# cvg/nicer-slam

Hardware: AMD Instinct MI355X
Metric: rays/sec (fwd+bwd), one tracking iteration (higher is better)
Workload: dtype f32; 1 GPU; Replica room0 tracking iteration, 1024 rays x 128 samples (+640 sampler evaluations/ray), single MI355X, fp32 [BASELINE configs[1]]; rays_per_gpu=1024, samples_per_ray=128, sampler_evals_per_ray=640, global_rays=1024, engine=fused, param_grads=False, hip_graph=True, driver=KernelTracker, python_gc=off inside the timed regions (as timeit), ray_chunks=1, cache_prewarm_steps=100, cache_prewarm_batches=disjoint from the warm-up and timed batches, parallelism=single, rccl_ranks=0, full=False

## Files before the change

### include/nicer_slam_amd.h

```cpp
#ifndef NICER_SLAM_AMD_H
#define NICER_SLAM_AMD_H

#include <stdint.h>

#ifdef __cplusplus
extern "C" {
#endif

#define NSA_OK 0
#define NSA_EUNSUPPORTED_C 1
#define NSA_ETOO_MANY_LEVELS 2
#define NSA_ELAUNCH 3
#define NSA_EBADARG 4
#define NSA_EUNSUPPORTED_NET 5
#define NSA_EMESH_TOO_LARGE 6

#define NSA_MAX_LEVELS 32

typedef void *nsa_stream_t;

const char *nsa_strerror(int code);
int nsa_version(void);


// ... 140 lines not shown
                   float beta1, float beta2, float eps, uint32_t lr_step, float lr_gamma, const float *loss, float *best,
                   nsa_stream_t stream);
int nsa_track_begin(const float *uv_in, const float *gt_in, float *uv, float *gt, const float *K, const float *cam, uint32_t n,
                    float *pose, float *rays_o, float *rays_d, float *depth_scale, nsa_stream_t stream);
int nsa_track_begin_draw(const float *uv_in, const float *gt_in, float *uv, float *gt, const float *K, const float *cam, uint32_t n,
                         float *pose, float *rays_o, float *rays_d, float *depth_scale, uint64_t *state, uint64_t n_rand,
                         float *t_rand, uint32_t E, uint32_t n_extra, uint32_t S, int32_t *extra_idx, nsa_stream_t stream);
int nsa_composite_track(const float *rays_o, const float *rays_d, const float *z_vals, const float *sdf, const float *rgb,
                        const float *voxels, uint32_t voxel_res, uint32_t R, uint32_t S, const float *gt, uint32_t n_total,
                        float *rgb_values, float *ray_loss, float *g_sdf, float *g_rgb, float *g_grad, nsa_stream_t stream);
int nsa_track_finish(const float *uv, const float *K, float *cam, uint32_t n, uint32_t S, const float *z_vals, const float *g_x,
                     const float *g_dir, const float *ray_loss, float *g_cam, int do_adam, float reduce_weight, float *exp_avg,
                     float *exp_avg_sq, float *step, float lr, float beta1, float beta2, float eps, uint32_t lr_step,
                     float lr_gamma, float *best, float *workspace, nsa_stream_t stream);
uint64_t nsa_track_finish_workspace(uint32_t n);
int nsa_adam_step_scaled(float *param, const float *grad, const float *grad_div, float *exp_avg, float *exp_avg_sq,
                         float *step, uint32_t n, float lr, float beta1, float beta2, float eps, uint32_t lr_step,
                         float lr_gamma, const float *loss, float *best, nsa_stream_t stream);


int nsa_morton_keys(const nsa_points_t *pts, int32_t *keys, nsa_stream_t stream);

int nsa_morton_order(const nsa_points_t *pts, int32_t *order, uint32_t *workspace, uint32_t key_bits, nsa_stream_t stream);
uint64_t nsa_morton_order_workspace(uint32_t P);

int nsa_update_voxels(const nsa_points_t *pts, float *voxels, uint32_t res, nsa_stream_t stream);

int nsa_adam_table_step(float *param, const float *grad, float *exp_avg, float *exp_avg_sq, uint64_t n, uint32_t step,
                        float lr, float beta1, float beta2, float eps, nsa_stream_t stream);

// ... 139 lines not shown
```

### nicer_slam_amd/_native.py

```python
import ctypes
import os

import torch

_TAG = os.environ.get("NSA_LIB_TAG", "")
_LIB_PATH = os.path.join(os.path.dirname(os.path.abspath(__file__)), "lib",
                         "libnicer_slam_amd" + ("_" + _TAG if _TAG else "") + ".so")

if not os.path.exists(_LIB_PATH):
    raise ImportError(
        f"{_LIB_PATH} not found: the HIP extension has not been built.  Run "
        "`python -m nicer_slam_amd.build` (needs hipcc; cross-compiles gfx950 without a GPU).")

lib = ctypes.CDLL(_LIB_PATH)

_p, _u32, _f32, _i = ctypes.c_void_p, ctypes.c_uint32, ctypes.c_float, ctypes.c_int

lib.nsa_strerror.restype = ctypes.c_char_p
lib.nsa_strerror.argtypes = [_i]
lib.nsa_version.restype = _i
lib.nsa_hash_encode_forward.restype = _i
lib.nsa_hash_encode_forward.argtypes = [_p, _p, _p, _p, _u32, _u32, _u32, _u32, _f32, _u32, _i, _p, _p]
lib.nsa_hash_encode_backward.restype = _i
lib.nsa_hash_encode_backward.argtypes = [_p, _p, _p, _p, _p, _u32, _u32, _u32, _u32, _f32, _u32, _i, _p, _p, _p]
# ... 179 lines not shown
lib.nsa_track_tail.argtypes = [_p, _p, _p, _u32, _p, _p, _p, _i, _f32, _p, _p, _p, _f32, _f32, _f32, _f32, _u32, _f32, _p, _p,
                               _p]
EXPORTS += ["nsa_track_head", "nsa_track_tail"]
lib.nsa_track_begin.restype = _i
lib.nsa_track_begin.argtypes = [_p, _p, _p, _p, _p, _p, _u32, _p, _p, _p, _p, _p]
lib.nsa_composite_track.restype = _i
lib.nsa_composite_track.argtypes = [_p, _p, _p, _p, _p, _p, _u32, _u32, _u32, _p, _u32, _p, _p, _p, _p, _p, _p]
lib.nsa_track_finish.restype = _i
lib.nsa_track_finish.argtypes = [_p, _p, _p, _u32, _u32, _p, _p, _p, _p, _p, _i, _f32, _p, _p, _p, _f32, _f32, _f32, _f32, _u32,
                                 _f32, _p, _p, _p]
lib.nsa_track_finish_workspace.restype = ctypes.c_uint64
lib.nsa_track_finish_workspace.argtypes = [_u32]
lib.nsa_track_begin_draw.restype = _i
lib.nsa_track_begin_draw.argtypes = [_p, _p, _p, _p, _p, _p, _u32, _p, _p, _p, _p, _p, ctypes.c_uint64, _p, _u32, _u32, _u32, _p, _p]
EXPORTS += ["nsa_track_begin", "nsa_track_begin_draw", "nsa_composite_track", "nsa_track_finish", "nsa_track_finish_workspace"]

lib.nsa_morton_keys.restype = _i
lib.nsa_morton_keys.argtypes = [_pp, _p, _p]
lib.nsa_morton_order.restype = _i
lib.nsa_morton_order.argtypes = [_pp, _p, _p, _u32, _p]
lib.nsa_morton_order_workspace.restype = ctypes.c_uint64
lib.nsa_morton_order_workspace.argtypes = [_u32]
EXPORTS += ["nsa_morton_order", "nsa_morton_order_workspace"]
EXPORTS += ["nsa_morton_keys"]

lib.nsa_adam_step_scaled.restype = _i
lib.nsa_adam_step_scaled.argtypes = [_p, _p, _p, _p, _p, _p, _u32, _f32, _f32, _f32, _f32, _u32, _f32, _p, _p, _p]
EXPORTS += ["nsa_adam_step_scaled"]


# ... 46 lines not shown
```

### nicer_slam_amd/csrc/render_sdfnet4.hip

```cpp
#include <cstdlib>
#include "sdf_net4.hpp"

namespace nsa {

#ifndef NSA_NW4_FWD
#define NSA_NW4_FWD 4
#endif
#ifndef NSA_NW4_BWD
#define NSA_NW4_BWD 8
#endif
#ifndef NSA_NW4_PAIR
#define NSA_NW4_PAIR 8
#endif
constexpr int stage_floats4(int nw) { return nw >= 8 ? 9216 : 6144; }

struct SdfNet4Args {
    PointSrc src;
    const float* table;
    const float* wp;
    float divide_factor;
    int accumulate;
    float* sdf;
    float* grad;
    float* feat;
// ... 282 lines not shown
    __shared__ LevelGeom s_geom[16];
    stage16_begin<Seq, Seq::NW, Seq::BUF>(stage, a.wp);
    geom_to_lds(geom, s_geom);
    const int lane = threadIdx.x & 63;
    const int j = lane & 15, q = lane >> 4;
    uint32_t tile = blockIdx.x * Seq::NW + (threadIdx.x >> 6);
    const uint32_t n_tiles = (a.src.P + 15) / 16;
    const bool wave_live = tile < n_tiles;
    if (!wave_live) tile = n_tiles - 1;
#define NSA_BODY_SYNC __syncthreads();
#include "sdfnet4_bwd_body.inc"
#undef NSA_BODY_SYNC
    TS_MARK(10)
    TS_END
}

static_assert(NSA_NW4_BWD * 64 * (2 * 8 + 1) <= stage_floats4(NSA_NW4_BWD), "scatter scratch must fit the idle stage buffer");

#if NSA_PIECES == 1
template <int LC, int CC, int NHC, int LF, int CF, int NHF>
__global__ __launch_bounds__(64 * NSA_NW4_PAIR, NSA_OCC4_FWD) void k_sdfnet4_fwd_pair_res(SdfNet4PairArgs a, GridGeom16 gc, GridGeom16 gf) {
    using Seq = ResidentSeq<SdfOpsPair<NHC, NHF>>;
    __shared__ __attribute__((aligned(16))) float stage[res_off<Seq>(Seq::n)];
    __shared__ LevelGeom s_geom[32];
    resident_load<Seq, Seq::NW>(stage, a.wp_c, a.wp_f);
    if (threadIdx.x < 16) s_geom[threadIdx.x] = gc.lv[threadIdx.x];
    else if (threadIdx.x < 32) s_geom[threadIdx.x] = gf.lv[threadIdx.x - 16];
    stage_wait();
    const int lane = threadIdx.x & 63;
    const int j = lane & 15, q = lane >> 4;
// ... 127 lines not shown
                           (hipStream_t)stream, a, gc, gf);
        return launch_end();
    }
#endif
    hipLaunchKernelGGL((k_sdfnet4_fwd_pair<4, 8, 1, 8, 4, 3>), dim3((tiles + NSA_NW4_PAIR - 1) / NSA_NW4_PAIR), dim3(64 * NSA_NW4_PAIR), 0,
                       (hipStream_t)stream, a, gc, gf);
    return launch_end();
}

#ifdef NSA_X_TS
int NSA_ENTRY(nsa_debug_set_ts)(unsigned long long* p) {
    return hipMemcpyToSymbol(HIP_SYMBOL(nsa::g_ts4), &p, sizeof(p)) == hipSuccess ? 0 : 3;
}
#endif

int NSA_ENTRY(nsa_sdfnet4_emit_rows)(uint32_t n_hidden) {
    return n_hidden == 1 ? nsa::SE4<1>::ROWS : n_hidden == 3 ? nsa::SE4<3>::ROWS : -1;
}

}
```

### nicer_slam_amd/csrc/sdfnet4_bwd_body.inc

```
    uint32_t pid = tile * 16 + j;
    const bool live = wave_live && pid < a.src.P;
    if (pid >= a.src.P) pid = a.src.P - 1;
    const uint32_t pt = point_of(a.src, pid);
    float x[3], z;
    uint32_t ray;
    load_point(a.src, pt, x, ray, z);
    NSA_BODY_SYNC
    TS_MARK(4)
    constexpr int kJac = (8 / C) * 3 * C;
    __shared__ float jac_lds[Seq::NW * kJac * 64];
    float* jstore = jac_lds + (threadIdx.x >> 6) * (kJac * 64) + lane;
    float in[QIN];
    pe_slots4(x, q, in);
    grid_slots4<L, C>(x, a.divide_factor, a.table, s_geom, q, in, jstore);
    const bool emit = MAP && a.emit != nullptr && wave_live;
    const Emitter4 em{emit ? a.emit + (size_t)tile * 16 + j : nullptr, a.emit_ld, live};
    float sg[NH][QHS], hl[QHS];
    TS_MARK(5)
    hidden_forward4<NH, Seq>(stage, 0, a.wp, lane, q, in, sg, hl, emit ? &em : nullptr);
    TS_MARK(6)
    float dh[NH > 1 ? NH - 1 : 1][QHS], dl[QIN];
    reverse_pass4<NH, Seq>(stage, NH, a.wp, lane, q, sg, dh, dl, emit ? &em : nullptr);
    TS_MARK(7)
    if (emit) {
// ... 89 lines not shown
    float hb0[QIN];
    {
        f32x4v a6[6];
#pragma unroll
        for (int t = 0; t < 6; ++t) a6[t] = f32x4v{0.0f, 0.0f, 0.0f, 0.0f};
        gemm16_staged<Seq, Seq::NW, Seq::BUF, 2, 6>(stage, a.wp, 4 * NH, lane, ab, a6, nullptr, &ab_bound);
#pragma unroll
        for (int s = 0; s < QIN; ++s) hb0[s] = a6[s >> 2][s & 3];
    }
    float gx[3];
    slots_to_x_jac4<L, C>(a.divide_factor, jstore, q, in, hb0, gx);
    constexpr int kIdle = (Seq::n_parts() - 1) & 1 ? 0 : 1;
    if (MAP && a.g_table)
        table_grad_scatter4<L, C>(x, a.divide_factor, s_geom, q, lane, live, hb0, dl, nbar, a.g_table,
                                  stage + kIdle * Seq::BUF + (threadIdx.x >> 6) * 64 * (2 * C + 1));
#pragma unroll
    for (int d = 0; d < 3; ++d) gx[d] = quad_sum(gx[d] + xb2[d]);
    if (live && q == 0) {
#pragma unroll
        for (int d = 0; d < 3; ++d) {
            float v = gx[d];
            if (a.accumulate) v += a.g_x[(size_t)pt * 3 + d];
            a.g_x[(size_t)pt * 3 + d] = v;
        }
    }
```

### nicer_slam_amd/csrc/track_tail.hip

```cpp
#include "grid_common.hpp"
#include "draw_common.hpp"

namespace nsa {

__device__ __forceinline__ void cam_to_pose(const float* __restrict__ q, float* __restrict__ P) {
    const float r = q[0], i = q[1], j = q[2], k = q[3];
    const float s = 2.0f / (r * r + i * i + j * j + k * k);
    P[0] = -s * (j * j + k * k) + 1.0f;  P[1] = s * (i * j - k * r);          P[2] = s * (i * k + j * r);           P[3] = q[4];
    P[4] = s * (i * j + k * r);          P[5] = -s * (i * i + k * k) + 1.0f;  P[6] = s * (j * k - i * r);           P[7] = q[5];
    P[8] = s * (i * k - j * r);          P[9] = s * (j * k + i * r);          P[10] = -s * (i * i + j * j) + 1.0f;  P[11] = q[6];
    P[12] = 0.0f; P[13] = 0.0f; P[14] = 0.0f; P[15] = 1.0f;
}

__global__ void k_cam_to_pose(const float* __restrict__ cam, float* __restrict__ pose, uint32_t b) {
    const uint32_t n = blockIdx.x * blockDim.x + threadIdx.x;
    if (n >= b) return;
    cam_to_pose(cam + 7 * n, pose + 16 * n);
}

__device__ __forceinline__ void pose_grad_to_cam(const float* __restrict__ q, const float* __restrict__ G, float* __restrict__ o) {
    const float r = q[0], i = q[1], j = q[2], k = q[3];
    const float nn = r * r + i * i + j * j + k * k;
    const float s = 2.0f / nn;
    const float N[9] = {-(j * j + k * k), i * j - k * r, i * k + j * r, i * j + k * r, -(i * i + k * k), j * k - i * r,
                        i * k - j * r, j * k + i * r, -(i * i + j * j)};
    float A = 0.0f;
#pragma unroll
// ... 99 lines not shown
}

struct TrackArgs {
    const float* uv;
    const float* K;
    float* cam;
    float* pose;
    uint32_t n;
    float* rays_o; float* rays_d; float* depth_scale;
    const float* g_o; const float* g_d;
    float* g_cam;
    float reduce_weight;
    AdamArgs adam;
};

__device__ __forceinline__ void lift_pixel_k(const float* __restrict__ K, float u, float v, float (&c)[3]) {
    const float fx = K[0], sk = K[1], cx = K[2], fy = K[5], cy = K[6];
    c[0] = (u - cx + cy * sk / fy - sk * v / fy) / fx;
    c[1] = (v - cy) / fy;
    c[2] = 1.0f;
}

__global__ __launch_bounds__(256) void k_track_head(TrackArgs a) {
    const uint32_t r = blockIdx.x * 256 + threadIdx.x;
    float P[16];
    cam_to_pose(a.cam, P);
    if (r == 0) {
#pragma unroll
        for (int i = 0; i < 16; ++i) a.pose[i] = P[i];
    }
    if (r >= a.n) return;
    float c[3];
    lift_pixel_k(a.K, a.uv[2 * r], a.uv[2 * r + 1], c);
    float v[3];
#pragma unroll
    for (int k = 0; k < 3; ++k) {
        const float w = P[4 * k] * c[0] + P[4 * k + 1] * c[1] + P[4 * k + 2] * c[2] + P[4 * k + 3];
// ... 73 lines not shown
    }
}

struct FinishArgs {
    TrackArgs t;
    const float* z_vals;
    const float* g_x;
    const float* g_dir;
    const float* ray_loss;
    uint32_t S;
    float inv_n;
    float* part;
    unsigned* ticket;
};

constexpr int FIN_Q = 13;

__device__ __forceinline__ void track_begin_block(const TrackArgs& a, const float* uv_in, const float* gt_in, float* uv, float* gt,
                                                  const uint32_t bid) {
    const uint32_t r = bid * 256 + threadIdx.x;
    float P[16];
    cam_to_pose(a.cam, P);
    if (r == 0) {
#pragma unroll
        for (int i = 0; i < 16; ++i) a.pose[i] = P[i];
    }
    if (r >= a.n) return;
    const float pu = uv_in[2 * r], pv = uv_in[2 * r + 1];
    uv[2 * r] = pu;
    uv[2 * r + 1] = pv;
#pragma unroll
    for (int k = 0; k < 3; ++k) gt[3 * r + k] = gt_in[3 * r + k];
// ... 8 lines not shown
    }
    const float s = v[0] * v[0] + v[1] * v[1] + v[2] * v[2];
#pragma unroll
    for (int k = 0; k < 3; ++k) a.rays_d[3 * r + k] = v[k] / s;
    a.depth_scale[r] = c[2] / (c[0] * c[0] + c[1] * c[1] + c[2] * c[2]);
}

__global__ __launch_bounds__(256) void k_track_begin(TrackArgs a, const float* uv_in, const float* gt_in, float* uv, float* gt) {
    track_begin_block(a, uv_in, gt_in, uv, gt, blockIdx.x);
}

__global__ __launch_bounds__(256) void k_track_begin_draw(TrackArgs a, const float* uv_in, const float* gt_in, float* uv, float* gt,
                                                          DrawArgs d, uint32_t begin_blocks) {
    if (blockIdx.x < begin_blocks) track_begin_block(a, uv_in, gt_in, uv, gt, blockIdx.x);
    else draw_block(d, blockIdx.x - begin_blocks, gridDim.x - begin_blocks);
}

constexpr int FIN_W = 16;

__global__ __launch_bounds__(64 * FIN_W) void k_track_finish(FinishArgs f) {
    __shared__ float rp[FIN_W][FIN_Q];
    __shared__ float G[16];
    __shared__ unsigned last;
    const TrackArgs& a = f.t;
    const int lane = threadIdx.x & 63, wv = threadIdx.x >> 6;
    const uint32_t ray = blockIdx.x * FIN_W + wv;
    float P[16];
    cam_to_pose(a.cam, P);
    float t0 = 0.0f, m0 = 0.0f, v0 = 0.0f, p0 = 0.0f;
    if (a.adam.p && threadIdx.x < 7) {
        t0 = a.adam.step[0];
        m0 = a.adam.m[threadIdx.x];
        v0 = a.adam.v[threadIdx.x];
        p0 = a.adam.p[threadIdx.x];
    }
    const float best0 = (a.adam.p && a.adam.best && threadIdx.x == 0) ? a.adam.best[0] : 0.0f;
    float vals[FIN_Q];
#pragma unroll
    for (int q = 0; q < FIN_Q; ++q) vals[q] = 0.0f;
    if (ray < a.n) {
        float acc[6] = {0, 0, 0, 0, 0, 0};
        for (uint32_t i = lane; i < f.S; i += 64) {
            const size_t p = (size_t)ray * f.S + i;
            const float z = f.z_vals[p];
#pragma unroll
            for (int c = 0; c < 3; ++c) {
                const float gx = f.g_x[p * 3 + c];
                acc[c] += gx;
                acc[3 + c] += z * gx + f.g_dir[p * 3 + c];
            }
        }
#pragma unroll
        for (int q = 0; q < 6; ++q) {
#pragma unroll
            for (int off = 32; off > 0; off >>= 1) acc[q] += __shfl_xor(acc[q], off);
        }
        float c[3], v[3];
        lift_pixel_k(a.K, a.uv[2 * ray], a.uv[2 * ray + 1], c);
#pragma unroll
        for (int k = 0; k < 3; ++k) {
            const float w = P[4 * k] * c[0] + P[4 * k + 1] * c[1] + P[4 * k + 2] * c[2] + P[4 * k + 3];
            v[k] = w - P[4 * k + 3];
        }
        const float s = v[0] * v[0] + v[1] * v[1] + v[2] * v[2];
        const float vg = v[0] * acc[3] + v[1] * acc[4] + v[2] * acc[5];
#pragma unroll
        for (int k = 0; k < 3; ++k) {
            const float vb = acc[3 + k] / s - 2.0f * v[k] * vg / (s * s);
#pragma unroll
            for (int j = 0; j < 3; ++j) vals[4 * k + j] = vb * c[j];
            vals[4 * k + 3] = acc[k];
        }
        vals[12] = f.ray_loss[ray];
    }
    if (lane == 0) {
#pragma unroll
        for (int q = 0; q < FIN_Q; ++q) rp[wv][q] = vals[q];
    }
    __syncthreads();
    if (wv == 0) {
        if (lane < FIN_Q) {
            float x = 0.0f;
#pragma unroll
            for (int w = 0; w < FIN_W; ++w) x += rp[w][lane];
            __hip_atomic_store(f.part + (size_t)blockIdx.x * 16 + lane, x, __ATOMIC_RELAXED, __HIP_MEMORY_SCOPE_AGENT);
        }
        __threadfence();
// ... 21 lines not shown
        }
        __syncthreads();
        if (lane == 0) {
#pragma unroll
            for (int q = 0; q < FIN_Q; ++q) rp[wv][q] = x[q];
        }
        __syncthreads();
        if (threadIdx.x < FIN_Q) {
            float g = 0.0f;
#pragma unroll
            for (int w = 0; w < FIN_W; ++w) g += rp[w][threadIdx.x];
            G[threadIdx.x] = g;
        }
    }
    __syncthreads();
    __shared__ float msg[9], stepped[8];
    if (threadIdx.x == 0) {
        f.ticket[0] = 0u;
        float o[8];
        pose_grad_to_cam(a.cam, G, o);
        o[7] = G[12] * f.inv_n;
        const float w = a.reduce_weight > 0.0f ? a.reduce_weight : 1.0f;
#pragma unroll
        for (int i = 0; i < 8; ++i) { msg[i] = o[i] * w; a.g_cam[i] = msg[i]; }
        if (a.reduce_weight > 0.0f) a.g_cam[8] = a.reduce_weight;
    }
    __syncthreads();
    if (a.adam.p) {
        const float t = t0 + 1.0f;
        if (threadIdx.x < 7) stepped[threadIdx.x] = adam_one(a.adam, threadIdx.x, t, m0, v0, p0, msg[threadIdx.x]);
        __syncthreads();
        if (threadIdx.x == 0) {
            a.adam.step[0] = t;
            if (a.adam.best && msg[7] < best0) {
                a.adam.best[0] = msg[7];
                for (int i = 0; i < 7; ++i) a.adam.best[1 + i] = stepped[i];
            }
        }
    }
}

}

extern "C" {

int nsa_cam_to_pose(const float* cam, uint32_t b, float* pose, nsa_stream_t stream) {
    using namespace nsa;
    if (b == 0) return NSA_OK;
    if (!cam || !pose) return NSA_EBADARG;
    launch_begin();
    hipLaunchKernelGGL(k_cam_to_pose, dim3((b + 63) / 64), dim3(64), 0, (hipStream_t)stream, cam, pose, b);
    return launch_end();
}

// ... 110 lines not shown
    FinishArgs f{};
    f.t.uv = uv; f.t.K = K; f.t.cam = cam; f.t.n = n; f.t.g_cam = g_cam; f.t.reduce_weight = reduce_weight;
    if (do_adam) f.t.adam = AdamArgs{cam, g_cam, exp_avg, exp_avg_sq, step, nullptr, 7, lr, beta1, beta2, eps, lr_gamma, lr_step,
                                      best, g_cam + 7, nullptr};
    f.z_vals = z_vals; f.g_x = g_x; f.g_dir = g_dir; f.ray_loss = ray_loss; f.S = S;
    f.inv_n = 1.0f / (float)(3 * (uint64_t)n);
    const uint32_t blocks = (n + FIN_W - 1) / FIN_W;
    f.ticket = reinterpret_cast<unsigned*>(workspace);
    f.part = workspace + 4;
    launch_begin();
    hipLaunchKernelGGL(k_track_finish, dim3(blocks), dim3(64 * FIN_W), 0, (hipStream_t)stream, f);
    return launch_end();
}

}
```

### nicer_slam_amd/fused/render.py

```python
import ctypes
import os

import torch

from .._native import lib, check, PointsDesc
from ..hashencoder.backend import _timed
from . import pack
from .sampler import COLOUR_COARSE_BWD, COLOUR_FWD_TRACK, forward_pair_ok, grid_desc, packed_sdf, precision_of, sdf_grid_desc, tile_of


def hl_size(P):
    return ((P + 31) // 32) * 2048


def save_size(P):
    return ((P + 31) // 32) * (4096 + 256)


def hl_index(P, device):
    pid = torch.arange(P, device=device).unsqueeze(1)
    f = torch.arange(64, device=device).unsqueeze(0)
    tile, p = pid // 32, pid % 32
    t, rho = f // 32, f % 32
    h = (rho >> 2) & 1
# ... 106 lines not shown
        return b
    with _timed("k_colour_fwd", P * 16 * 8 * 2 * 4):
        check(lib.nsa_colour_forward(ctypes.byref(pts), ctypes.byref(gr), pr.data_ptr(), b["grad"].data_ptr(),
                                     b["feat"].data_ptr(), b["rgb"].data_ptr(),
                                     b["save"].data_ptr() if need_bwd else None, st))
    if not composite:
        return b
    with _timed("k_composite_fwd", P * 32):
        check(lib.nsa_composite_forward(rays_o.data_ptr(), rays_d.data_ptr(), z_vals.data_ptr(), b["sdf"].data_ptr(),
                                        b["rgb"].data_ptr(), b["grad"].data_ptr(), b["vox"].data_ptr(), model.voxel_res,
                                        R, S, b["weights"].data_ptr(), b["rgb_values"].data_ptr(), b["depth"].data_ptr(),
                                        b["nmap"].data_ptr(), b["entropy"].data_ptr(), st))
    return b


def composite_backward_raw(model, rays_o, rays_d, z_vals, b, stage, color_stage, g_rgbv=None, g_depth=None, g_nmap=None,
                           g_ent=None, g_w=None, params=None, track=None, reduce_rays=True):
    R, S = z_vals.shape
    P = R * S
    dev = z_vals.device
    imp = model.implicit_network
    gc, keep_c = sdf_grid_desc(model, "coarse")
    gf, keep_f = sdf_grid_desc(model, "fine")
    gr, keep_r = grid_desc(model.rendering_network.encoding, model.rendering_network.divide_factor, 2, precision_of(model, "colour"))
    pc, pf, pr = b["packs"]
    order = b.get("order")
    pts = _pts(rays_o, rays_d, z_vals, order)
    st = _stream()
    ptr = lambda t: None if t is None else t.data_ptr()
    gs = [None if g is None else g.contiguous() for g in (g_rgbv, g_depth, g_nmap, g_ent, g_w)]
    done = b.get("track_out") if track is not None else None
    g_sdf = done["g_sdf"] if done else torch.empty(P, device=dev)
    g_rgb = done["g_rgb"] if done else torch.empty(P, 3, device=dev)
    g_grad = done["g_grad"] if done else torch.empty(P, 3, device=dev)
    if done:
        pass
    elif track is not None:
        with _timed("k_composite_track", P * 60):
            check(lib.nsa_composite_track(rays_o.data_ptr(), rays_d.data_ptr(), z_vals.data_ptr(), b["sdf"].data_ptr(),
                                          b["rgb"].data_ptr(), b["vox"].data_ptr(), model.voxel_res, R, S, track["gt"].data_ptr(),
                                          R, b["rgb_values"].data_ptr(), track["ray_loss"].data_ptr(), g_sdf.data_ptr(),
                                          g_rgb.data_ptr(), g_grad.data_ptr(), st))
    else:
        with _timed("k_composite_bwd", P * 60):
            check(lib.nsa_composite_backward(rays_o.data_ptr(), rays_d.data_ptr(), z_vals.data_ptr(), b["sdf"].data_ptr(),
                                             b["rgb"].data_ptr(), b["grad"].data_ptr(), b["vox"].data_ptr(), model.voxel_res,
# ... 56 lines not shown
        if want.get("tab_f") or want.get("flat_f"):
            from . import mapping
            enc = imp.fine.encoding
            gt = _table_grad(enc.embeddings) if want.get("tab_f") else None
            emit = (mapping.new_emit(mapping.se_rows(3, tile_of(model, "fine"))["ROWS"], P, dev, extra=2)
                    if want.get("flat_f") else None)
            with _timed("k_sdfnet_bwd<fine,map>", P * 3 * 8 * 8 * 4 * 4):
                check(lib.nsa_sdfnet_backward_params(ctypes.byref(pts), ctypes.byref(gf), pf.data_ptr(), g_sdf.data_ptr(),
                                                     g_feat.data_ptr(), g_grad.data_ptr(), 1, g_x.data_ptr(),
                                                     ptr(gt), ptr(emit), 0 if emit is None else emit.shape[1], st))
            if emit is not None:
                pg["flat_f"] = mapping.sdf_flat_grad(emit, g_sdf, P, enc.num_levels, enc.level_dim, NH=3,
                                                     tile=tile_of(model, "fine"), order=order)
                del emit
            pg["tab_f"] = _table_result(gt)
        else:
            with _timed("k_sdfnet_bwd<fine>", P * 3 * 8 * 8 * 4 * 4):
                check(lib.nsa_sdfnet_backward(ctypes.byref(pts), ctypes.byref(gf), pf.data_ptr(), g_sdf.data_ptr(),
                                              g_feat.data_ptr(), g_grad.data_ptr(), 1, g_x.data_ptr(), st))
    if "_keep" in b:
        b["_keep"].update(g_x=g_x, g_dir=g_dir, g_sdf=g_sdf, g_rgb=g_rgb, g_grad=g_grad, g_feat=g_feat)
    if not reduce_rays:
        return g_x, g_dir
    g_o = torch.empty(R, 3, device=dev)
    g_d = torch.empty(R, 3, device=dev)
    check(lib.nsa_rays_backward(z_vals.data_ptr(), g_x.data_ptr(), g_dir.data_ptr(), R, S, g_o.data_ptr(),
                                g_d.data_ptr(), st))
    if params is not None:
        return g_o, g_d, pg
    return g_o, g_d
# ... 59 lines not shown
```

### nicer_slam_amd/tracking.py

```python
import torch

from .dist import allreduce_pose_grad
from .hashencoder.backend import _timed
from .utils.general import get_camera_from_tensor


class KernelTracker:

    def __init__(self, model, intrinsics, n_rays, cam_init, lr=0.005, betas=(0.9, 0.999), eps=1e-8, lr_step=0,
                 lr_gamma=1.0, use_graph=True, world=1, stage="fine", color_stage="highfreq", chunks=1, graph_collective=None,
                 fold=True, draw_in_begin=True):
        from .fused import render as fr, sampler as fs
        if not fr.supported(model):
            raise RuntimeError("KernelTracker: configuration outside the fused engine's compiled set")
        dev = model.voxels.device
        self.fr, self.fs = fr, fs
        self.model, self.world, self.R = model, world, n_rays
        self.K = intrinsics.contiguous()
        self.stage, self.color_stage = stage, color_stage
        self.hyper = (float(lr), float(betas[0]), float(betas[1]), float(eps), int(lr_step), float(lr_gamma))
        self.cam = cam_init.detach().clone().to(dev).float().contiguous()
        self.uv = torch.zeros(1, n_rays, 2, device=dev)
        self.gt = torch.zeros(n_rays, 3, device=dev)
        self._uv_shape, self._gt_shape = (1, n_rays, 2), (n_rays, 3)
# ... 3 lines not shown
        self.best = z(8)
        self.best[0] = 1e10
        self.rays_o, self.rays_d, self.ds = z(n_rays, 3), z(n_rays, 3), z(n_rays)
        self.g_rgbv = z(n_rays, 3)
        import os
        if graph_collective is None:
            graph_collective = os.environ.get("NSA_GRAPH_COLLECTIVE", "0") == "1"
        self.collective_in_graph = bool(graph_collective and use_graph and world > 1)
        self.chunks = max(1, min(int(chunks), n_rays))
        if self.chunks > 1:
            from .dist import shard_rays
            self.bounds = [shard_rays(n_rays, c, self.chunks) for c in range(self.chunks)]
            self.streams = [torch.cuda.Stream() for _ in range(self.chunks)]
            self.red_c, self.pose_c = z(self.chunks, 9), z(self.chunks, 4, 4)
        self.folded = self.chunks == 1 and bool(fold)
        if self.folded:
            from ._native import lib
            self.ray_loss = z(n_rays)
            self.fin_ws = z(int(lib.nsa_track_finish_workspace(n_rays)))
        self.drawn = None
        if self.folded and draw_in_begin:
            samp = model.ray_sampler
            E, n_extra = samp.N_samples_eval, samp.N_samples_extra
            if E <= 1024:
                self.drawn = (torch.empty(n_rays, E, device=dev),
                              torch.empty(max(n_extra, 1), device=dev, dtype=torch.int32)[:n_extra] if n_extra > 0 else None)
        self._drawn_now = False
        self.graph = None
        self._began = False
        if use_graph:
# ... 27 lines not shown
        from ._native import lib, check
        fr, fs, model = self.fr, self.fs, self.model
        st = torch.cuda.current_stream().cuda_stream
        R = hi - lo
        uv, gt, g_rgbv = self.uv[0, lo:hi], self.gt[lo:hi], self.g_rgbv[lo:hi]
        rays_o, rays_d, ds = self.rays_o[lo:hi], self.rays_d[lo:hi], self.ds[lo:hi]
        lr, b1, b2, eps, lr_step, lr_gamma = self.hyper
        fused = not self.message
        if self.folded:
            if not self._began and not torch.cuda.is_current_stream_capturing():
                raise RuntimeError("KernelTracker: the folded sequence needs _begin() (nsa_track_begin) in front of every iteration -- "
                                   "the rays of the updated camera are lifted there, not inside the graph; use step()")
            self._began = False
            z_vals, _ = fs.get_z_vals(model, rays_d, rays_o, need_eik=False, rows=(lo, hi),
                                      drawn=self.drawn if self._drawn_now else None)
            trk = dict(gt=gt, ray_loss=self.ray_loss)
            b = fr.composite_forward_raw(model, rays_o, rays_d, z_vals, self.stage, True, composite=False, track=trk)
            g_x, g_dir = fr.composite_backward_raw(model, rays_o, rays_d, z_vals, b, self.stage, self.color_stage,
                                                   track=trk, reduce_rays=False)
            with _timed("k_track_finish", R * z_vals.shape[1] * 24):
                check(lib.nsa_track_finish(uv.data_ptr(), self.K.data_ptr(), self.cam.data_ptr(), R, z_vals.shape[1],
                                           z_vals.data_ptr(), g_x.data_ptr(), g_dir.data_ptr(), self.ray_loss.data_ptr(),
                                           red.data_ptr(), 1 if fused else 0, 0.0 if fused else float(R), self.m.data_ptr(),
                                           self.v.data_ptr(), self.t.data_ptr(), lr, b1, b2, eps, lr_step, lr_gamma,
                                           self.best.data_ptr() if fused else None, self.fin_ws.data_ptr(), st))
            return
        check(lib.nsa_track_head(uv.data_ptr(), self.K.data_ptr(), self.cam.data_ptr(), R, pose.data_ptr(),
                                 rays_o.data_ptr(), rays_d.data_ptr(), ds.data_ptr(), st))
        z_vals, _ = fs.get_z_vals(model, rays_d, rays_o, need_eik=False, rows=(lo, hi))
        b = fr.composite_forward_raw(model, rays_o, rays_d, z_vals, self.stage, True)
        check(lib.nsa_l1_loss(b["rgb_values"].data_ptr(), gt.data_ptr(), 3 * R, red[7:8].data_ptr(), g_rgbv.data_ptr(), st))
        g_o, g_d = fr.composite_backward_raw(model, rays_o, rays_d, z_vals, b, self.stage, self.color_stage, g_rgbv=g_rgbv)
        check(lib.nsa_track_tail(uv.data_ptr(), self.K.data_ptr(), self.cam.data_ptr(), R, g_o.data_ptr(),
                                 g_d.data_ptr(), red.data_ptr(), 1 if fused else 0, 0.0 if fused else float(R),
# ... 210 lines not shown
```

Before: 1.994 million rays/s.

## Fold per-ray pose gradient reduction into SDF backward kernel and single-block tail

Adds a tracking variant of the fine SDF-net backward kernel that reduces g_x and g_dir over each ray's samples inside the kernel and emits per-ray pose-gradient terms, or per-segment partials when a ray spans several blocks. A new single-block tail kernel sums these partials and runs the Adam step, replacing nsa_track_finish. The aim is to avoid re-reading per-sample g_x/g_dir arrays and the multi-block finish reduction. It adds block-level syncs and shared-memory reductions to the backward kernel, plus a per-iteration partials allocation.

```diff
diff --git a/include/nicer_slam_amd.h b/include/nicer_slam_amd.h
--- a/include/nicer_slam_amd.h
+++ b/include/nicer_slam_amd.h
@@ -178,6 +178,15 @@
                      float *exp_avg_sq, float *step, float lr, float beta1, float beta2, float eps, uint32_t lr_step,
                      float lr_gamma, float *best, float *workspace, nsa_stream_t stream);
 uint64_t nsa_track_finish_workspace(uint32_t n);
+int nsa_sdfnet_backward_track(const nsa_points_t *pts, const nsa_grid_t *grid, const float *packed, const float *g_sdf,
+                              const float *g_feat_hl, const float *g_grad, int accumulate, float *g_x, const float *g_dir,
+                              const float *uv, const float *K, const float *cam, const float *ray_loss, float *partials,
+                              nsa_stream_t stream);
+int nsa_track_fold_tail(const float *uv, const float *K, float *cam, uint32_t n, uint32_t S, const float *partials,
+                        const float *ray_loss, float *g_cam, int do_adam, float reduce_weight, float *exp_avg, float *exp_avg_sq,
+                        float *step, float lr, float beta1, float beta2, float eps, uint32_t lr_step, float lr_gamma, float *best,
+                        nsa_stream_t stream);
+uint64_t nsa_track_fold_workspace(uint32_t n, uint32_t S);
 int nsa_adam_step_scaled(float *param, const float *grad, const float *grad_div, float *exp_avg, float *exp_avg_sq,
                          float *step, uint32_t n, float lr, float beta1, float beta2, float eps, uint32_t lr_step,
                          float lr_gamma, const float *loss, float *best, nsa_stream_t stream);
diff --git a/nicer_slam_amd/_native.py b/nicer_slam_amd/_native.py
--- a/nicer_slam_amd/_native.py
+++ b/nicer_slam_amd/_native.py
@@ -217,6 +217,14 @@
 lib.nsa_track_begin_draw.restype = _i
 lib.nsa_track_begin_draw.argtypes = [_p, _p, _p, _p, _p, _p, _u32, _p, _p, _p, _p, _p, ctypes.c_uint64, _p, _u32, _u32, _u32, _p, _p]
 EXPORTS += ["nsa_track_begin", "nsa_track_begin_draw", "nsa_composite_track", "nsa_track_finish", "nsa_track_finish_workspace"]
+lib.nsa_sdfnet_backward_track.restype = _i
+lib.nsa_sdfnet_backward_track.argtypes = [_pp, _gp, _p, _p, _p, _p, _i, _p, _p, _p, _p, _p, _p, _p, _p]
+lib.nsa_track_fold_tail.restype = _i
+lib.nsa_track_fold_tail.argtypes = [_p, _p, _p, _u32, _u32, _p, _p, _p, _i, _f32, _p, _p, _p, _f32, _f32, _f32, _f32, _u32, _f32,
+                                    _p, _p]
+lib.nsa_track_fold_workspace.restype = ctypes.c_uint64
+lib.nsa_track_fold_workspace.argtypes = [_u32, _u32]
+EXPORTS += ["nsa_sdfnet_backward_track", "nsa_track_fold_tail", "nsa_track_fold_workspace"]
 
 lib.nsa_morton_keys.restype = _i
 lib.nsa_morton_keys.argtypes = [_pp, _p, _p]
diff --git a/nicer_slam_amd/csrc/render_sdfnet4.hip b/nicer_slam_amd/csrc/render_sdfnet4.hip
--- a/nicer_slam_amd/csrc/render_sdfnet4.hip
+++ b/nicer_slam_amd/csrc/render_sdfnet4.hip
@@ -1,5 +1,6 @@
 #include <cstdlib>
 #include "sdf_net4.hpp"
+#include "track_common.hpp"
 
 namespace nsa {
 
@@ -320,6 +321,114 @@
     TS_MARK(10)
     TS_END
 }
+
+
+#if NSA_PIECES != 1
+struct TrackFold {
+    const float* g_dir;
+    const float* uv;
+    const float* K;
+    const float* cam;
+    const float* ray_loss;
+    float* part;
+    int per_ray;
+};
+
+template <int L, int C, int NH>
+__global__ __launch_bounds__(64 * NSA_NW4_BWD, NSA_OCC4_BWD) void k_sdfnet4_bwd_track(SdfNet4Args a, GridGeom16 geom, TrackFold tf) {
+    constexpr bool MAP = false;
+    using P = SdfPack4<NH>;
+    using Seq = SdfOps4<NH, true>;
+    using E = SE4<NH>;
+    __shared__ __attribute__((aligned(16))) float stage[2 * Seq::BUF];
+    __shared__ LevelGeom s_geom[16];
+    __shared__ float wave_sums[Seq::NW][6];
+    stage16_begin<Seq, Seq::NW, Seq::BUF>(stage, a.wp);
+    geom_to_lds(geom, s_geom);
+    const int lane = threadIdx.x & 63;
+    const int j = lane & 15, q = lane >> 4;
+    uint32_t tile = blockIdx.x * Seq::NW + (threadIdx.x >> 6);
+    const uint32_t n_tiles = (a.src.P + 15) / 16;
+    const bool wave_live = tile < n_tiles;
+    if (!wave_live) tile = n_tiles - 1;
+    float gdir[3] = {0.0f, 0.0f, 0.0f}, zt = 0.0f;
+    float camv[7], Kv[7], uv[2], rl = 0.0f;
+#define NSA_BWD_TAIL_LOADS                                                                                          \
+    if (live && q == 0) {                                                                                           \
+        zt = a.src.z_vals[pt];                                                                                      \
+        for (int d = 0; d < 3; ++d) gdir[d] = tf.g_dir[(size_t)pt * 3 + d];                                         \
+    }                                                                                                               \
+    if (tf.per_ray && threadIdx.x == 0) {                                                                           \
+        for (int i = 0; i < 7; ++i) { camv[i] = tf.cam[i]; Kv[i] = tf.K[i]; }                                        \
+        uv[0] = tf.uv[2 * ray]; uv[1] = tf.uv[2 * ray + 1];                                                          \
+        rl = tf.ray_loss[ray];                                                                                      \
+    }
+#define NSA_BODY_SYNC __syncthreads();
+#pragma push_macro("TS_MARK")
+#undef TS_MARK
+#define TS_MARK(slot)
+#include "sdfnet4_bwd_body.inc"
+#pragma pop_macro("TS_MARK")
+#undef NSA_BODY_SYNC
+#undef NSA_BWD_TAIL_LOADS
+    const bool on = live && q == 0;
+    float sv[6];
+#pragma unroll
+    for (int d = 0; d < 3; ++d) {
+        sv[d] = on ? gx[d] : 0.0f;
+        sv[3 + d] = on ? zt * gx[d] + gdir[d] : 0.0f;
+    }
+    if (tf.per_ray) {
+#pragma unroll
+        for (int k = 0; k < 6; ++k) {
+#pragma unroll
+            for (int off = 8; off > 0; off >>= 1) sv[k] += __shfl_xor(sv[k], off);
+        }
+        if (lane == 0) {
+#pragma unroll
+            for (int k = 0; k < 6; ++k) wave_sums[threadIdx.x >> 6][k] = sv[k];
+        }
+        __syncthreads();
+        if (threadIdx.x == 0) {
+            float go[3] = {0.0f, 0.0f, 0.0f}, gd[3] = {0.0f, 0.0f, 0.0f};
+#pragma unroll
+            for (int w = 0; w < Seq::NW; ++w) {
+#pragma unroll
+                for (int d = 0; d < 3; ++d) {
+                    go[d] += wave_sums[w][d];
+                    gd[d] += wave_sums[w][3 + d];
+                }
+            }
+            float Pm[16], c[3], vals[FIN_Q];
+            cam_to_pose(camv, Pm);
+            lift_pixel_k(Kv, uv[0], uv[1], c);
+            ray_pose_terms(Pm, c, go, gd, vals);
+            vals[12] = rl;
+#pragma unroll
+            for (int k = 0; k < FIN_Q; ++k) tf.part[(size_t)ray * 16 + k] = vals[k];
+        }
+    } else {
+        const int up = (lane + 63) & 63;
+        const uint32_t ray_prev = __shfl(ray, up);
+#pragma unroll
+        for (int off = 1; off < 16; off <<= 1) {
+            const int src = (lane + off) & 63;
+            const uint32_t ray_src = __shfl(ray, src);
+            const bool take = j + off < 16 && ray_src == ray;
+#pragma unroll
+            for (int k = 0; k < 6; ++k) {
+                const float o = __shfl(sv[k], src);
+                sv[k] += take ? o : 0.0f;
+            }
+        }
+        if (on && (j == 0 || ray_prev != ray)) {
+#pragma unroll
+            for (int k = 0; k < 6; ++k) tf.part[(size_t)pid * 8 + k] = sv[k];
+        }
+    }
+}
+
+#endif
 
 static_assert(NSA_NW4_BWD * 64 * (2 * 8 + 1) <= stage_floats4(NSA_NW4_BWD), "scatter scratch must fit the idle stage buffer");
 
@@ -477,6 +586,34 @@
 }
 #endif
 
+#if NSA_PIECES != 1
+int nsa_sdfnet_backward_track(const nsa_points_t* pts, const nsa_grid_t* grid, const float* packed, const float* g_sdf,
+                              const float* g_feat_hl, const float* g_grad, int accumulate, float* g_x, const float* g_dir,
+                              const float* uv, const float* K, const float* cam, const float* ray_loss, float* partials,
+                              nsa_stream_t stream) {
+    using namespace nsa;
+    if (!pts || !grid || !packed || !g_x || !g_dir || !uv || !K || !cam || !ray_loss || !partials) return NSA_EBADARG;
+    if (pts->points || pts->order || !pts->rays_o || !pts->rays_d || !pts->z_vals || pts->S == 0 || pts->P == 0 ||
+        pts->P % pts->S != 0)
+        return NSA_EBADARG;
+    if (grid->precision != 0 || grid->tile != 16 || !(grid->L == 8 && grid->C == 4 && grid->n_hidden == 3)) return NSA_EUNSUPPORTED_NET;
+    const int per_ray = pts->S == kFoldRayS;
+    if (per_ray && 16 * NSA_NW4_BWD != (int)kFoldRayS) return NSA_EUNSUPPORTED_NET;
+    SdfNet4Args a{};
+    a.src = PointSrc{pts->rays_o, pts->rays_d, pts->z_vals, nullptr, pts->P, pts->S, nullptr};
+    a.table = grid->table; a.wp = packed; a.divide_factor = grid->divide_factor; a.accumulate = accumulate;
+    a.g_sdf = g_sdf; a.g_feat = g_feat_hl; a.g_grad = g_grad; a.g_x = g_x;
+    const TrackFold tf{g_dir, uv, K, cam, ray_loss, partials, per_ray};
+    GridGeom16 geom;
+    if (int rc = make_grid_geom16(grid->offsets_host, grid->L, grid->S, grid->H, &geom, grid->C)) return rc;
+    const uint32_t tiles = (pts->P + 15) / 16;
+    launch_begin();
+    hipLaunchKernelGGL((k_sdfnet4_bwd_track<8, 4, 3>), dim3((tiles + NSA_NW4_BWD - 1) / NSA_NW4_BWD), dim3(64 * NSA_NW4_BWD), 0,
+                       (hipStream_t)stream, a, geom, tf);
+    return launch_end();
+}
+#endif
+
 int NSA_ENTRY(nsa_sdfnet4_emit_rows)(uint32_t n_hidden) {
     return n_hidden == 1 ? nsa::SE4<1>::ROWS : n_hidden == 3 ? nsa::SE4<3>::ROWS : -1;
 }
diff --git a/nicer_slam_amd/csrc/sdfnet4_bwd_body.inc b/nicer_slam_amd/csrc/sdfnet4_bwd_body.inc
--- a/nicer_slam_amd/csrc/sdfnet4_bwd_body.inc
+++ b/nicer_slam_amd/csrc/sdfnet4_bwd_body.inc
@@ -127,13 +127,15 @@
     if (MAP && a.g_table)
         table_grad_scatter4<L, C>(x, a.divide_factor, s_geom, q, lane, live, hb0, dl, nbar, a.g_table,
                                   stage + kIdle * Seq::BUF + (threadIdx.x >> 6) * 64 * (2 * C + 1));
+#ifdef NSA_BWD_TAIL_LOADS
+    NSA_BWD_TAIL_LOADS
+#endif
 #pragma unroll
     for (int d = 0; d < 3; ++d) gx[d] = quad_sum(gx[d] + xb2[d]);
     if (live && q == 0) {
 #pragma unroll
         for (int d = 0; d < 3; ++d) {
-            float v = gx[d];
-            if (a.accumulate) v += a.g_x[(size_t)pt * 3 + d];
-            a.g_x[(size_t)pt * 3 + d] = v;
+            if (a.accumulate) gx[d] += a.g_x[(size_t)pt * 3 + d];
+            a.g_x[(size_t)pt * 3 + d] = gx[d];
         }
     }
diff --git a/nicer_slam_amd/csrc/track_common.hpp b/nicer_slam_amd/csrc/track_common.hpp
--- /dev/null
+++ b/nicer_slam_amd/csrc/track_common.hpp
@@ -0,0 +1,46 @@
+#pragma once
+#include <hip/hip_runtime.h>
+#include <stdint.h>
+
+namespace nsa {
+
+__device__ __forceinline__ void cam_to_pose(const float* __restrict__ q, float* __restrict__ P) {
+    const float r = q[0], i = q[1], j = q[2], k = q[3];
+    const float s = 2.0f / (r * r + i * i + j * j + k * k);
+    P[0] = -s * (j * j + k * k) + 1.0f;  P[1] = s * (i * j - k * r);          P[2] = s * (i * k + j * r);           P[3] = q[4];
+    P[4] = s * (i * j + k * r);          P[5] = -s * (i * i + k * k) + 1.0f;  P[6] = s * (j * k - i * r);           P[7] = q[5];
+    P[8] = s * (i * k - j * r);          P[9] = s * (j * k + i * r);          P[10] = -s * (i * i + j * j) + 1.0f;  P[11] = q[6];
+    P[12] = 0.0f; P[13] = 0.0f; P[14] = 0.0f; P[15] = 1.0f;
+}
+
+__device__ __forceinline__ void lift_pixel_k(const float* __restrict__ K, float u, float v, float (&c)[3]) {
+    const float fx = K[0], sk = K[1], cx = K[2], fy = K[5], cy = K[6];
+    c[0] = (u - cx + cy * sk / fy - sk * v / fy) / fx;
+    c[1] = (v - cy) / fy;
+    c[2] = 1.0f;
+}
+
+constexpr uint32_t kFoldRayS = 128;
+
+constexpr int FIN_Q = 13;
+
+__device__ __forceinline__ void ray_pose_terms(const float (&P)[16], const float (&c)[3], const float (&g_o)[3], const float (&g_d)[3],
+                                               float (&vals)[FIN_Q]) {
+    float v[3];
+#pragma unroll
+    for (int k = 0; k < 3; ++k) {
+        const float w = P[4 * k] * c[0] + P[4 * k + 1] * c[1] + P[4 * k + 2] * c[2] + P[4 * k + 3];
+        v[k] = w - P[4 * k + 3];
+    }
+    const float s = v[0] * v[0] + v[1] * v[1] + v[2] * v[2];
+    const float vg = v[0] * g_d[0] + v[1] * g_d[1] + v[2] * g_d[2];
+#pragma unroll
+    for (int k = 0; k < 3; ++k) {
+        const float vb = g_d[k] / s - 2.0f * v[k] * vg / (s * s);
+#pragma unroll
+        for (int j = 0; j < 3; ++j) vals[4 * k + j] = vb * c[j];
+        vals[4 * k + 3] = g_o[k];
+    }
+}
+
+}
diff --git a/nicer_slam_amd/csrc/track_tail.hip b/nicer_slam_amd/csrc/track_tail.hip
--- a/nicer_slam_amd/csrc/track_tail.hip
+++ b/nicer_slam_amd/csrc/track_tail.hip
@@ -1,16 +1,8 @@
 #include "grid_common.hpp"
 #include "draw_common.hpp"
+#include "track_common.hpp"
 
 namespace nsa {
-
-__device__ __forceinline__ void cam_to_pose(const float* __restrict__ q, float* __restrict__ P) {
-    const float r = q[0], i = q[1], j = q[2], k = q[3];
-    const float s = 2.0f / (r * r + i * i + j * j + k * k);
-    P[0] = -s * (j * j + k * k) + 1.0f;  P[1] = s * (i * j - k * r);          P[2] = s * (i * k + j * r);           P[3] = q[4];
-    P[4] = s * (i * j + k * r);          P[5] = -s * (i * i + k * k) + 1.0f;  P[6] = s * (j * k - i * r);           P[7] = q[5];
-    P[8] = s * (i * k - j * r);          P[9] = s * (j * k + i * r);          P[10] = -s * (i * i + j * j) + 1.0f;  P[11] = q[6];
-    P[12] = 0.0f; P[13] = 0.0f; P[14] = 0.0f; P[15] = 1.0f;
-}
 
 __global__ void k_cam_to_pose(const float* __restrict__ cam, float* __restrict__ pose, uint32_t b) {
     const uint32_t n = blockIdx.x * blockDim.x + threadIdx.x;
@@ -140,13 +132,6 @@
     AdamArgs adam;
 };
 
-__device__ __forceinline__ void lift_pixel_k(const float* __restrict__ K, float u, float v, float (&c)[3]) {
-    const float fx = K[0], sk = K[1], cx = K[2], fy = K[5], cy = K[6];
-    c[0] = (u - cx + cy * sk / fy - sk * v / fy) / fx;
-    c[1] = (v - cy) / fy;
-    c[2] = 1.0f;
-}
-
 __global__ __launch_bounds__(256) void k_track_head(TrackArgs a) {
     const uint32_t r = blockIdx.x * 256 + threadIdx.x;
     float P[16];
@@ -250,8 +235,6 @@
     unsigned* ticket;
 };
 
-constexpr int FIN_Q = 13;
-
 __device__ __forceinline__ void track_begin_block(const TrackArgs& a, const float* uv_in, const float* gt_in, float* uv, float* gt,
                                                   const uint32_t bid) {
     const uint32_t r = bid * 256 + threadIdx.x;
@@ -290,6 +273,47 @@
                                                           DrawArgs d, uint32_t begin_blocks) {
     if (blockIdx.x < begin_blocks) track_begin_block(a, uv_in, gt_in, uv, gt, blockIdx.x);
     else draw_block(d, blockIdx.x - begin_blocks, gridDim.x - begin_blocks);
+}
+
+struct StepState {
+    float t0, m0, v0, p0, best0;
+    __device__ __forceinline__ static StepState load(const TrackArgs& a) {
+        StepState s{0.0f, 0.0f, 0.0f, 0.0f, 0.0f};
+        if (a.adam.p && threadIdx.x < 7) {
+            s.t0 = a.adam.step[0];
+            s.m0 = a.adam.m[threadIdx.x];
+            s.v0 = a.adam.v[threadIdx.x];
+            s.p0 = a.adam.p[threadIdx.x];
+        }
+        if (a.adam.p && a.adam.best && threadIdx.x == 0) s.best0 = a.adam.best[0];
+        return s;
+    }
+};
+
+__device__ __forceinline__ void track_step(const TrackArgs& a, const float* G, float inv_n, const StepState& st) {
+    __shared__ float msg[9], stepped[8];
+    if (threadIdx.x == 0) {
+        float o[8];
+        pose_grad_to_cam(a.cam, G, o);
+        o[7] = G[12] * inv_n;
+        const float w = a.reduce_weight > 0.0f ? a.reduce_weight : 1.0f;
+#pragma unroll
+        for (int i = 0; i < 8; ++i) { msg[i] = o[i] * w; a.g_cam[i] = msg[i]; }
+        if (a.reduce_weight > 0.0f) a.g_cam[8] = a.reduce_weight;
+    }
+    __syncthreads();
+    if (a.adam.p) {
+        const float t = st.t0 + 1.0f;
+        if (threadIdx.x < 7) stepped[threadIdx.x] = adam_one(a.adam, threadIdx.x, t, st.m0, st.v0, st.p0, msg[threadIdx.x]);
+        __syncthreads();
+        if (threadIdx.x == 0) {
+            a.adam.step[0] = t;
+            if (a.adam.best && msg[7] < st.best0) {
+                a.adam.best[0] = msg[7];
+                for (int i = 0; i < 7; ++i) a.adam.best[1 + i] = stepped[i];
+            }
+        }
+    }
 }
 
 constexpr int FIN_W = 16;
@@ -303,14 +327,7 @@
     const uint32_t ray = blockIdx.x * FIN_W + wv;
     float P[16];
     cam_to_pose(a.cam, P);
-    float t0 = 0.0f, m0 = 0.0f, v0 = 0.0f, p0 = 0.0f;
-    if (a.adam.p && threadIdx.x < 7) {
-        t0 = a.adam.step[0];
-        m0 = a.adam.m[threadIdx.x];
-        v0 = a.adam.v[threadIdx.x];
-        p0 = a.adam.p[threadIdx.x];
-    }
-    const float best0 = (a.adam.p && a.adam.best && threadIdx.x == 0) ? a.adam.best[0] : 0.0f;
+    const StepState st = StepState::load(a);
     float vals[FIN_Q];
 #pragma unroll
     for (int q = 0; q < FIN_Q; ++q) vals[q] = 0.0f;
@@ -331,22 +348,9 @@
 #pragma unroll
             for (int off = 32; off > 0; off >>= 1) acc[q] += __shfl_xor(acc[q], off);
         }
-        float c[3], v[3];
+        float c[3];
         lift_pixel_k(a.K, a.uv[2 * ray], a.uv[2 * ray + 1], c);
-#pragma unroll
-        for (int k = 0; k < 3; ++k) {
-            const float w = P[4 * k] * c[0] + P[4 * k + 1] * c[1] + P[4 * k + 2] * c[2] + P[4 * k + 3];
-            v[k] = w - P[4 * k + 3];
-        }
-        const float s = v[0] * v[0] + v[1] * v[1] + v[2] * v[2];
-        const float vg = v[0] * acc[3] + v[1] * acc[4] + v[2] * acc[5];
-#pragma unroll
-        for (int k = 0; k < 3; ++k) {
-            const float vb = acc[3 + k] / s - 2.0f * v[k] * vg / (s * s);
-#pragma unroll
-            for (int j = 0; j < 3; ++j) vals[4 * k + j] = vb * c[j];
-            vals[4 * k + 3] = acc[k];
-        }
+        ray_pose_terms(P, c, {acc[0], acc[1], acc[2]}, {acc[3], acc[4], acc[5]}, vals);
         vals[12] = f.ray_loss[ray];
     }
     if (lane == 0) {
@@ -398,30 +402,69 @@
         }
     }
     __syncthreads();
-    __shared__ float msg[9], stepped[8];
-    if (threadIdx.x == 0) {
-        f.ticket[0] = 0u;
-        float o[8];
-        pose_grad_to_cam(a.cam, G, o);
-        o[7] = G[12] * f.inv_n;
-        const float w = a.reduce_weight > 0.0f ? a.reduce_weight : 1.0f;
-#pragma unroll
-        for (int i = 0; i < 8; ++i) { msg[i] = o[i] * w; a.g_cam[i] = msg[i]; }
-        if (a.reduce_weight > 0.0f) a.g_cam[8] = a.reduce_weight;
-    }
-    __syncthreads();
-    if (a.adam.p) {
-        const float t = t0 + 1.0f;
-        if (threadIdx.x < 7) stepped[threadIdx.x] = adam_one(a.adam, threadIdx.x, t, m0, v0, p0, msg[threadIdx.x]);
-        __syncthreads();
-        if (threadIdx.x == 0) {
-            a.adam.step[0] = t;
-            if (a.adam.best && msg[7] < best0) {
-                a.adam.best[0] = msg[7];
-                for (int i = 0; i < 7; ++i) a.adam.best[1 + i] = stepped[i];
+    if (threadIdx.x == 0) f.ticket[0] = 0u;
+    track_step(a, G, f.inv_n, st);
+}
+
+__global__ __launch_bounds__(1024) void k_track_fold_tail(FinishArgs f, int per_ray) {
+    __shared__ float rp[16][FIN_Q];
+    __shared__ float G[16];
+    const TrackArgs& a = f.t;
+    const int lane = threadIdx.x & 63, wv = threadIdx.x >> 6;
+    const StepState st = StepState::load(a);
+    float x[FIN_Q];
+#pragma unroll
+    for (int q = 0; q < FIN_Q; ++q) x[q] = 0.0f;
+    if (per_ray) {
+        for (uint32_t r = threadIdx.x; r < a.n; r += 1024) {
+            float v[FIN_Q];
+#pragma unroll
+            for (int q = 0; q < FIN_Q; ++q) v[q] = f.part[(size_t)r * 16 + q];
+#pragma unroll
+            for (int q = 0; q < FIN_Q; ++q) x[q] += v[q];
+        }
+    } else {
+        float P[16];
+        cam_to_pose(a.cam, P);
+        for (uint32_t r = threadIdx.x; r < a.n; r += 1024) {
+            float go[3] = {0.0f, 0.0f, 0.0f}, gd[3] = {0.0f, 0.0f, 0.0f};
+            const size_t p0 = (size_t)r * f.S, t0 = p0 / 16;
+            const uint32_t n_seg = (uint32_t)((p0 + f.S - 1) / 16 - t0 + 1);
+#pragma unroll 4
+            for (uint32_t i = 0; i < n_seg; ++i) {
+                const size_t p = i == 0 ? p0 : (t0 + i) * 16;
+#pragma unroll
+                for (int c = 0; c < 3; ++c) {
+                    go[c] += f.part[p * 8 + c];
+                    gd[c] += f.part[p * 8 + 3 + c];
+                }
             }
-        }
-    }
+            float c[3], v[FIN_Q];
+            lift_pixel_k(a.K, a.uv[2 * r], a.uv[2 * r + 1], c);
+            ray_pose_terms(P, c, go, gd, v);
+            v[12] = f.ray_loss[r];
+#pragma unroll
+            for (int q = 0; q < FIN_Q; ++q) x[q] += v[q];
+        }
+    }
+#pragma unroll
+    for (int q = 0; q < FIN_Q; ++q) {
+#pragma unroll
+        for (int off = 32; off > 0; off >>= 1) x[q] += __shfl_xor(x[q], off);
+    }
+    if (lane == 0) {
+#pragma unroll
+        for (int q = 0; q < FIN_Q; ++q) rp[wv][q] = x[q];
+    }
+    __syncthreads();
+    if (threadIdx.x < FIN_Q) {
+        float g = 0.0f;
+#pragma unroll
+        for (int w = 0; w < 16; ++w) g += rp[w][threadIdx.x];
+        G[threadIdx.x] = g;
+    }
+    __syncthreads();
+    track_step(a, G, f.inv_n, st);
 }
 
 }
@@ -562,3 +605,31 @@
 }
 
 }
+
+extern "C" {
+
+uint64_t nsa_track_fold_workspace(uint32_t n, uint32_t S) {
+    return S == nsa::kFoldRayS ? (uint64_t)n * 16 : (uint64_t)n * S * 8;
+}
+
+int nsa_track_fold_tail(const float* uv, const float* K, float* cam, uint32_t n, uint32_t S, const float* partials,
+                        const float* ray_loss, float* g_cam, int do_adam, float reduce_weight, float* exp_avg, float* exp_avg_sq,
+                        float* step, float lr, float beta1, float beta2, float eps, uint32_t lr_step, float lr_gamma, float* best,
+                        nsa_stream_t stream) {
+    using namespace nsa;
+    if (!uv || !K || !cam || !partials || !ray_loss || !g_cam || n == 0 || S == 0) return NSA_EBADARG;
+    if (do_adam && (!exp_avg || !exp_avg_sq || !step)) return NSA_EBADARG;
+    if (best && !do_adam) return NSA_EBADARG;
+    FinishArgs f{};
+    f.t.uv = uv; f.t.K = K; f.t.cam = cam; f.t.n = n; f.t.g_cam = g_cam; f.t.reduce_weight = reduce_weight;
+    if (do_adam) f.t.adam = AdamArgs{cam, g_cam, exp_avg, exp_avg_sq, step, nullptr, 7, lr, beta1, beta2, eps, lr_gamma, lr_step,
+                                      best, g_cam + 7, nullptr};
+    f.ray_loss = ray_loss; f.S = S;
+    f.inv_n = 1.0f / (float)(3 * (uint64_t)n);
+    f.part = const_cast<float*>(partials);
+    launch_begin();
+    hipLaunchKernelGGL(k_track_fold_tail, dim3(1), dim3(1024), 0, (hipStream_t)stream, f, S == kFoldRayS ? 1 : 0);
+    return launch_end();
+}
+
+}
diff --git a/nicer_slam_amd/fused/render.py b/nicer_slam_amd/fused/render.py
--- a/nicer_slam_amd/fused/render.py
+++ b/nicer_slam_amd/fused/render.py
@@ -144,6 +144,10 @@
     return b
 
 
+def track_fold_supported(grid):
+    return grid.tile == 16 and grid.precision == 0 and (grid.L, grid.C, grid.n_hidden) == (8, 4, 3)
+
+
 def composite_backward_raw(model, rays_o, rays_d, z_vals, b, stage, color_stage, g_rgbv=None, g_depth=None, g_nmap=None,
                            g_ent=None, g_w=None, params=None, track=None, reduce_rays=True):
     R, S = z_vals.shape
@@ -160,6 +164,9 @@
     ptr = lambda t: None if t is None else t.data_ptr()
     gs = [None if g is None else g.contiguous() for g in (g_rgbv, g_depth, g_nmap, g_ent, g_w)]
     done = b.get("track_out") if track is not None else None
+    fold = track.get("fold") if track is not None else None
+    if fold is not None:
+        fold["done"] = False
     g_sdf = done["g_sdf"] if done else torch.empty(P, device=dev)
     g_rgb = done["g_rgb"] if done else torch.empty(P, 3, device=dev)
     g_grad = done["g_grad"] if done else torch.empty(P, 3, device=dev)
@@ -246,6 +253,13 @@
                                                      tile=tile_of(model, "fine"), order=order)
                 del emit
             pg["tab_f"] = _table_result(gt)
+        elif fold is not None and track_fold_supported(gf) and order is None:
+            with _timed("k_sdfnet_bwd<fine>", P * 3 * 8 * 8 * 4 * 4):
+                check(lib.nsa_sdfnet_backward_track(ctypes.byref(pts), ctypes.byref(gf), pf.data_ptr(), g_sdf.data_ptr(),
+                                                    g_feat.data_ptr(), g_grad.data_ptr(), 1, g_x.data_ptr(), g_dir.data_ptr(),
+                                                    fold["uv"].data_ptr(), fold["K"].data_ptr(), fold["cam"].data_ptr(),
+                                                    track["ray_loss"].data_ptr(), fold["partials"].data_ptr(), st))
+            fold["done"] = True
         else:
             with _timed("k_sdfnet_bwd<fine>", P * 3 * 8 * 8 * 4 * 4):
                 check(lib.nsa_sdfnet_backward(ctypes.byref(pts), ctypes.byref(gf), pf.data_ptr(), g_sdf.data_ptr(),
diff --git a/nicer_slam_amd/tracking.py b/nicer_slam_amd/tracking.py
--- a/nicer_slam_amd/tracking.py
+++ b/nicer_slam_amd/tracking.py
@@ -41,6 +41,7 @@
             self.streams = [torch.cuda.Stream() for _ in range(self.chunks)]
             self.red_c, self.pose_c = z(self.chunks, 9), z(self.chunks, 4, 4)
         self.folded = self.chunks == 1 and bool(fold)
+        self.tail_folded = False
         if self.folded:
             from ._native import lib
             self.ray_loss = z(n_rays)
@@ -98,10 +99,22 @@
             self._began = False
             z_vals, _ = fs.get_z_vals(model, rays_d, rays_o, need_eik=False, rows=(lo, hi),
                                       drawn=self.drawn if self._drawn_now else None)
-            trk = dict(gt=gt, ray_loss=self.ray_loss)
+            S = z_vals.shape[1]
+            partials = torch.empty(int(lib.nsa_track_fold_workspace(R, S)), device=z_vals.device)
+            fold = dict(uv=uv, K=self.K, cam=self.cam, partials=partials)
+            trk = dict(gt=gt, ray_loss=self.ray_loss, fold=fold)
             b = fr.composite_forward_raw(model, rays_o, rays_d, z_vals, self.stage, True, composite=False, track=trk)
             g_x, g_dir = fr.composite_backward_raw(model, rays_o, rays_d, z_vals, b, self.stage, self.color_stage,
                                                    track=trk, reduce_rays=False)
+            self.tail_folded = fold["done"]
+            if fold["done"]:
+                with _timed("k_track_finish", R * 64):
+                    check(lib.nsa_track_fold_tail(uv.data_ptr(), self.K.data_ptr(), self.cam.data_ptr(), R, S, partials.data_ptr(),
+                                                  self.ray_loss.data_ptr(), red.data_ptr(), 1 if fused else 0,
+                                                  0.0 if fused else float(R), self.m.data_ptr(), self.v.data_ptr(),
+                                                  self.t.data_ptr(), lr, b1, b2, eps, lr_step, lr_gamma,
+                                                  self.best.data_ptr() if fused else None, st))
+                return
             with _timed("k_track_finish", R * z_vals.shape[1] * 24):
                 check(lib.nsa_track_finish(uv.data_ptr(), self.K.data_ptr(), self.cam.data_ptr(), R, z_vals.shape[1],
                                            z_vals.data_ptr(), g_x.data_ptr(), g_dir.data_ptr(), self.ray_loss.data_ptr(),
```

Result: no change. 1.997 million rays/s (median of 6 runs) (+0.2%).
